# starkware-libs/stark-perpetual

Measured on AMD Instinct MI355X. Metric: pedersen_hashes_per_sec, higher is better.
Workload: dtype u32x9; 1 GPU; 2^16-leaf Pedersen Merkle rebuild per GPU (BASELINE.json configs[1]), 63 rebuilds in lockstep; tree_height=16, leaves_per_gpu=65536, calls_per_region=28, streams=2, window_bits=26, combine=none

## Files before the change

### stark-perpetual_amd/csrc/pedersen.hip

```cpp
#include <algorithm>
#include <cstdlib>
#include <cstring>
#include <map>
#include <vector>

#include "context.hpp"
#include "pedersen.hpp"
#include "quad.hpp"
#include "ragged_plan.hpp"

#ifndef SP_ACC_WAVES
#define SP_ACC_WAVES 1
#endif

namespace sp {

struct raw_aff {
  u256 x, y;
};
__device__ __forceinline__ raw_aff ld_raw(const aff_packed* e) {
  const uint4* q = reinterpret_cast<const uint4*>(e);
  const uint4 a = q[0], b = q[1], c = q[2], d = q[3];
  raw_aff r;
  r.x.w[0] = a.x; r.x.w[1] = a.y; r.x.w[2] = a.z; r.x.w[3] = a.w;
// ... 173 lines not shown
                      const int2* __restrict__ src, size_t plane) {
  bulk_accumulate(x, y, xstride, ystride, n, ped, w0, log2e, nwin, sX, sZZ, status, flag, src, plane,
                  (size_t)blockIdx.x * blockDim.x + threadIdx.x);
}

__device__ __forceinline__ fe shfl_xor_fe(const fe& v, int mask) {
  fe r;
#pragma unroll
  for (int i = 0; i < NL; ++i) r.l[i] = __shfl_xor(v.l[i], mask, 64);
  return r;
}
__device__ __forceinline__ uint32_t field_from_memory(const uint64_t* felt, int bit, int width) {
  const uint32_t* w = reinterpret_cast<const uint32_t*>(felt);
  const int wi = bit >> 5, sh = bit & 31;
  uint64_t two = (uint64_t)w[wi];
  if (wi + 1 < 8) two |= (uint64_t)w[wi + 1] << 32;
  return (uint32_t)(two >> sh) & ((1u << width) - 1u);
}
__device__ __forceinline__ uint32_t window_from_memory(const uint64_t* fx, const uint64_t* fy, int start,
                                                       int width) {
  if (start + width <= 252) return field_from_memory(fx, start, width);
  if (start >= 252) return field_from_memory(fy, start - 252, width);
  const int lo_n = 252 - start;
  return field_from_memory(fx, start, lo_n) | (field_from_memory(fy, 0, width - lo_n) << lo_n);
}

template <int LOG_L>
__device__ __forceinline__ xyzz split_accumulate(const uint64_t* fx, const uint64_t* fy, int sub,
                                                 const aff_packed* __restrict__ ped, int w0, int log2e,
                                                 int nwin) {
  constexpr int L = 1 << LOG_L;
  const int cnt_lo = nwin / L, extra = nwin % L;
  const int cnt = cnt_lo + (sub < extra ? 1 : 0);
  const int g0 = sub * cnt_lo + (sub < extra ? sub : extra);
  auto entry = [&](int g) {
    return window_entry(ped, g, window_from_memory(fx, fy, window_start(g, w0, log2e), window_width(g, w0, log2e)),
                        w0, log2e);
  };
  const window_ref r0 = entry(g0);
  const aff q0 = signed_aff(ld_raw(r0.entry), r0.negative);
  window_ref rn = entry(g0 + 1);
  raw_aff nxt = ld_raw(rn.entry);
  xyzz acc;
  {
    const aff q1 = signed_aff(nxt, rn.negative);
    if (cnt > 2) {
      rn = entry(g0 + 2);
      nxt = ld_raw(rn.entry);
    }
    acc = xyzz_mmadd<SP_SCAN_SPLIT>(q0, q1);
  }
  for (int j = 2; j < cnt; ++j) {
    const aff q = signed_aff(nxt, rn.negative);
    if (j + 1 < cnt) {
      rn = entry(g0 + j + 1);
      nxt = ld_raw(rn.entry);
    }
    acc = xyzz_madd<SP_SCAN_SPLIT>(acc, q);
  }
#pragma unroll 1
  for (int r = 0; r + 1 < LOG_L; ++r) {
    xyzz o;
    o.X = shfl_xor_fe(acc.X, 1 << r);
    o.Y = shfl_xor_fe(acc.Y, 1 << r);
    o.ZZ = shfl_xor_fe(acc.ZZ, 1 << r);
    o.ZZZ = shfl_xor_fe(acc.ZZZ, 1 << r);
    acc = xyzz_add<SP_SCAN_SPLIT>(acc, o);
  }
  if constexpr (LOG_L > 0) {
    constexpr int r = LOG_L - 1;
    xyzz o;
    o.X = shfl_xor_fe(acc.X, 1 << r);
    o.Y = shfl_xor_fe(acc.Y, 1 << r);
    o.ZZ = shfl_xor_fe(acc.ZZ, 1 << r);
    o.ZZZ = shfl_xor_fe(acc.ZZZ, 1 << r);
    fe X3, ZZ3;
    xyzz_add_x_only<SP_SCAN_SPLIT>(acc, o, X3, ZZ3);
    acc.X = X3;
    acc.ZZ = ZZ3;
  }
  return acc;
}

template <int LOG_L, bool FUSED>
__global__ void __launch_bounds__(256)
ped_accumulate_split_kernel(const uint64_t* __restrict__ x, const uint64_t* __restrict__ y, size_t xstride,
                            size_t ystride, size_t n, const aff_packed* __restrict__ ped, int w0, int log2e,
                            int nwin, int32_t* __restrict__ sX, int32_t* __restrict__ sZZ,
                            uint8_t* __restrict__ status, unsigned* __restrict__ flag,
                            const int2* __restrict__ src, uint64_t* __restrict__ out, size_t ostride,
                            size_t plane) {
  constexpr int L = 1 << LOG_L;
  const size_t gt = (size_t)blockIdx.x * blockDim.x + threadIdx.x;
  const size_t e_raw = gt >> LOG_L;
  const int sub = (int)(gt & (L - 1));
  const bool active = e_raw < n;
  const size_t e = active ? e_raw : n - 1;
  const uint64_t *fx, *fy;
  operand_pointers(x, y, xstride, ystride, src, e, fx, fy);
  const xyzz acc = split_accumulate<LOG_L>(fx, fy, sub, ped, w0, log2e, nwin);
  uint8_t st = SP_HASH_OK;
  u256 xa_plain;
  if (FUSED) {
    fe zz = acc.ZZ;
    if constexpr (LOG_L < 2) {
      if (fe_is_zero(zz)) {
        zz = FE_ONE_M;
        st = SP_HASH_UNHASHABLE;
      }
    }
    const fe zinv = fe_inv_shared_quad<(LOG_L >= 2 ? 0 : 2 - LOG_L), true>(zz, (int)(threadIdx.x & 3));
    if constexpr (LOG_L >= 2) {
      if (limbs_is_zero(zinv)) st = SP_HASH_UNHASHABLE;
    }
    xa_plain = fe_pack(fe_canon(fe_mul(acc.X, zinv)));
  }
  if (!active || sub != 0) return;
  if (!u256_lt(ld_u256(fx), U256_P) || !u256_lt(ld_u256(fy), U256_P)) st = SP_HASH_OUT_OF_RANGE;
  if (FUSED) {
    st_u256(out + 4 * e * ostride, xa_plain);
  } else {
    store_limbs(sX, plane, e, acc.X);
    store_limbs(sZZ, plane, e, acc.ZZ);
  }
  if (status) status[e] = st;
  if (st != SP_HASH_OK && flag) atomicOr(flag, (unsigned)st);
}

template <int LOG_L>
__global__ void __launch_bounds__(256, SP_ACC_WAVES)
ped_accumulate_mixed_kernel(const uint64_t* __restrict__ x, const uint64_t* __restrict__ y, size_t xstride,
                            size_t ystride, size_t n_bulk, size_t rem, unsigned bulk_blocks,
                            const aff_packed* __restrict__ ped, int w0, int log2e, int nwin,
                            int32_t* __restrict__ sX, int32_t* __restrict__ sZZ, uint8_t* __restrict__ status,
                            unsigned* __restrict__ flag, const int2* __restrict__ src, size_t plane) {
  if (blockIdx.x < bulk_blocks) {
    bulk_accumulate(x, y, xstride, ystride, n_bulk, ped, w0, log2e, nwin, sX, sZZ, status, flag, src, plane,
                    (size_t)blockIdx.x * blockDim.x + threadIdx.x);
    return;
  }
  constexpr int L = 1 << LOG_L;
  const size_t gt = (size_t)(blockIdx.x - bulk_blocks) * blockDim.x + threadIdx.x;
  const size_t e_raw = gt >> LOG_L;
  const int sub = (int)(gt & (L - 1));
  const bool active = e_raw < rem;
  const size_t e = n_bulk + (active ? e_raw : rem - 1);
  const uint64_t *fx, *fy;
  operand_pointers(x, y, xstride, ystride, src, e, fx, fy);
  const xyzz acc = split_accumulate<LOG_L>(fx, fy, sub, ped, w0, log2e, nwin);
  if (!active || sub != 0) return;
  uint8_t st = SP_HASH_OK;
  if (!u256_lt(ld_u256(fx), U256_P) || !u256_lt(ld_u256(fy), U256_P)) st = SP_HASH_OUT_OF_RANGE;
  store_limbs(sX, plane, e, acc.X);
  store_limbs(sZZ, plane, e, acc.ZZ);
  if (status) status[e] = st;
  if (st != SP_HASH_OK && flag) atomicOr(flag, (unsigned)st);
}

template <int LOG_Q, bool SPARSE>
__device__ __forceinline__ u256 quad_hash(const uint64_t* fx, const uint64_t* fy, int mode, const aff_packed* __restrict__ cpts,
                                          int cx, int cy, const aff_packed* __restrict__ ped, int w0, int log2e,
                                          int nwin_plan, int g, bool* unhashable) {
  constexpr int QUADS = 1 << LOG_Q;
  const int q = g >> 2, k = g & 3;
  int nwin = nwin_plan, first_real = 0;
  if constexpr (SPARSE) {
    nwin = mode == 0 ? nwin_plan : 1 + nwin_plan - (mode == 1 ? cx : cy);
    first_real = mode == 1 ? cx - 1 : (mode == 2 ? -1 : 0);
  }
  auto entry = [&](int v) {
    if constexpr (SPARSE) {
      if (mode != 0 && v == 0) return unpack_raw(ld_raw(cpts + (mode - 1)));
    }
    const int w = first_real + v;
    const window_ref r =
        window_entry(ped, w, window_from_memory(fx, fy, window_start(w, w0, log2e), window_width(w, w0, log2e)), w0, log2e);
    return signed_aff(ld_raw(r.entry), r.negative);
  };
  const int cnt = nwin / QUADS + (q < nwin % QUADS ? 1 : 0);
  int max_cnt = (nwin + QUADS - 1) / QUADS;
  if constexpr (SPARSE) {
    max_cnt = 0;
    if (__any(mode == 0)) max_cnt = (nwin_plan + QUADS - 1) / QUADS;
    if (__any(mode == 1)) max_cnt = max(max_cnt, (1 + nwin_plan - cx + QUADS - 1) / QUADS);
    if (__any(mode == 2)) max_cnt = max(max_cnt, (1 + nwin_plan - cy + QUADS - 1) / QUADS);
  }
  const bool upper = (k & 2) != 0;
  const bool odd = (k & 1) != 0;
  const int wa = (upper && cnt >= 3) ? q + 2 * QUADS : q;
  const int wb = (upper && cnt >= 4) ? q + 3 * QUADS : q + QUADS;
  const aff pa = entry(wa), pb = entry(wb);
  qpt p = qmmadd(pa.x, pa.y, pb.x, pb.y, k);
  if (upper && cnt == 3) {
    p.a = odd ? pa.y : pa.x;
    p.b = FE_ONE_M;
  }
  qpt s = qadd<false>(p, k);
  if (cnt == 2) {
    s.a = fe_dpp<quad_perm(0, 1, 0, 1)>(p.a);
// ... 194 lines not shown
    const u256 xa = quad_hash<LOG_Q, false>(fx, fy, 0, nullptr, 0, 0, ped, w0, log2e, nwin_plan, g, &unhashable);
    if (live && g == 0) {
      if (!u256_lt(ld_u256(w), U256_P) || (j == 0 && !u256_lt(ld_u256(h), U256_P))) st |= SP_HASH_OUT_OF_RANGE;
      else if (unhashable) st |= SP_HASH_UNHASHABLE;
    }
    __syncthreads();
    if (live && g == 0) {
      uint32_t* sl = reinterpret_cast<uint32_t*>(slot[grp]);
#pragma unroll
      for (int k = 0; k < 8; ++k) sl[k] = xa.w[k];
      if (j == steps - 1 && writer) {
        fold_result<SIDED>(e, xa, st, out, status, expect, estride, verdict);
        if (st != SP_HASH_OK && flag) atomicOr(flag, (unsigned)st);
      }
    }
    __syncthreads();
    h = slot[grp];
  }
}

__global__ void __launch_bounds__(256)
ped_fold_ragged_scatter_kernel(const uint64_t* __restrict__ work, const uint64_t* __restrict__ lone, bool sided,
                               const uint32_t* __restrict__ off, const uint32_t* __restrict__ perm,
                               const uint32_t* __restrict__ step_off, const uint8_t* __restrict__ step_status, size_t n,
                               unsigned* __restrict__ flag, uint8_t* __restrict__ status, uint64_t* __restrict__ out,
                               const uint64_t* __restrict__ expect, size_t estride, uint8_t* __restrict__ verdict) {
  const size_t k = (size_t)blockIdx.x * blockDim.x + threadIdx.x;
  if (k >= n) return;
  const uint32_t c = perm[k];
  const uint32_t o0 = off[c], steps = off[c + 1] - o0 - (sided ? 0 : 1);
  uint8_t st = SP_HASH_OK;
  u256 v;
  if (steps == 0) {
    v = ld_u256(lone + 4 * (size_t)(sided ? c : o0));
    if (!u256_lt(v, U256_P)) st = SP_HASH_OUT_OF_RANGE;
    if (st != SP_HASH_OK && flag) atomicOr(flag, (unsigned)st);
  } else {
    v = ld_u256(work + 4 * k);
    for (uint32_t s = 0; s < steps; ++s) st |= step_status[(size_t)step_off[s] + k];
  }
  fold_result<true>(c, v, st, out, status, expect, estride, verdict);
}

__global__ void __launch_bounds__(256)
ped_top_kernel(uint64_t* __restrict__ cur, size_t n_in, int n_levels, const aff_packed* __restrict__ ped, int w0, int log2e,
               int nwin_plan, unsigned* __restrict__ flag) {
  constexpr int LANES = 32, GROUPS = 256 / LANES;
  __shared__ uint64_t slot[2][GROUPS][4];
  const int g = (int)(threadIdx.x % LANES), grp = (int)(threadIdx.x / LANES);
  const size_t b = blockIdx.x;
  const int chunk = 1 << n_levels;
  uint64_t* out = cur + 4 * n_in;
  size_t n_out = n_in >> 1;
  int share = 4 - n_levels;
  for (int t = 0; t < n_levels; ++t, ++share) {
    const int cnt = chunk >> (t + 1);
    const int i = grp >> share;
    const bool writer = g == 0 && (grp & ((1 << share) - 1)) == 0;
    const uint64_t *fx, *fy;
    if (t == 0) {
      fx = cur + 4 * ((size_t)chunk * b + 2 * (size_t)i);
      fy = fx + 4;
    } else {
      fx = slot[(t - 1) & 1][2 * i];
      fy = slot[(t - 1) & 1][2 * i + 1];
    }
    bool unhashable;
    const u256 xa = quad_hash<3, false>(fx, fy, 0, nullptr, 0, 0, ped, w0, log2e, nwin_plan, g, &unhashable);
    uint8_t st = unhashable ? SP_HASH_UNHASHABLE : SP_HASH_OK;
    if (t == 0 && writer && (!u256_lt(ld_u256(fx), U256_P) || !u256_lt(ld_u256(fy), U256_P))) st = SP_HASH_OUT_OF_RANGE;
    if (writer) {
      uint32_t* sl = reinterpret_cast<uint32_t*>(slot[t & 1][i]);
#pragma unroll
      for (int w = 0; w < 8; ++w) sl[w] = xa.w[w];
      st_u256(out + 4 * ((size_t)cnt * b + (size_t)i), xa);
      if (st != SP_HASH_OK && flag) atomicOr(flag, (unsigned)st);
    }
    __syncthreads();
    out += 4 * n_out;
    n_out >>= 1;
  }
}

__global__ void __launch_bounds__(256)
ped_finish_kernel(const int32_t* __restrict__ sX, int32_t* __restrict__ sZZ, int32_t* __restrict__ sPre,
                  size_t n, size_t T, uint64_t* __restrict__ out, size_t ostride,
                  uint8_t* __restrict__ status, unsigned* __restrict__ flag) {
  const size_t t = (size_t)blockIdx.x * blockDim.x + threadIdx.x;
  if (t >= T) return;
  const size_t cnt = t < n ? (n - t + T - 1) / T : 0;
  fe run = FE_ONE_M;
  if (cnt > 0) {
    fe znext = load_limbs(sZZ, n, t);
#pragma unroll 1
    for (size_t j = 0; j < cnt; ++j) {
      const size_t e = t + j * T;
      const fe z = znext;
      if (j + 1 < cnt) znext = load_limbs(sZZ, n, e + T);
      store_limbs(sPre, n, e, run);
      run = fe_mul(run, z);
    }
  }
  if (fe_is_zero(run)) {
    run = FE_ONE_M;
#pragma unroll 1
    for (size_t e = t; e < n; e += T) {
      fe z = load_limbs(sZZ, n, e);
      if (fe_is_zero(z)) {
        z = FE_ONE_M;
        store_limbs(sZZ, n, e, z);
        if (status) status[e] = SP_HASH_UNHASHABLE;
        if (flag) atomicOr(flag, (unsigned)SP_HASH_UNHASHABLE);
      }
      store_limbs(sPre, n, e, run);
      run = fe_mul(run, z);
    }
  }
  size_t e = cnt > 0 ? t + (cnt - 1) * T : 0;
  fe zn = run, pn = run, xn = run;
  if (cnt > 0) {
    zn = load_limbs(sZZ, n, e);
    pn = load_limbs(sPre, n, e);
    xn = load_limbs(sX, n, e);
  }
  fe inv = fe_inv_shared_quad<2, true>(run, (int)(threadIdx.x & 3));
#pragma unroll 1
  for (size_t j = cnt; j-- > 0;) {
    const fe z = zn, pre = pn, xv = xn;
    const size_t cur = t + j * T;
    if (j > 0) {
      zn = load_limbs(sZZ, n, cur - T);
      pn = load_limbs(sPre, n, cur - T);
      xn = load_limbs(sX, n, cur - T);
    }
    const fe zinv = fe_mul(inv, pre);
    inv = fe_mul(inv, z);
    const fe xa = fe_mul(xv, zinv);
    st_u256(out + 4 * cur * ostride, fe_pack(fe_canon(xa)));
  }
}

template <bool Z_IN_LDS>
__global__ void __launch_bounds__(256)
ped_finish_lds_kernel(const int32_t* __restrict__ sX, int32_t* __restrict__ sZZ, size_t n, size_t T,
                      uint64_t* __restrict__ out, size_t ostride, uint8_t* __restrict__ status,
                      unsigned* __restrict__ flag, int kmax) {
  extern __shared__ int32_t fin_lds[];
  int32_t* lpre = fin_lds;
  int32_t* lz = fin_lds + (size_t)kmax * NL * 256;
  auto lds_put = [&](int32_t* base, size_t j, const fe& v) {
#pragma unroll
    for (int k = 0; k < NL; ++k) base[((j * NL + k) << 8) + threadIdx.x] = v.l[k];
  };
  auto lds_get = [&](const int32_t* base, size_t j) {
    fe v;
#pragma unroll
    for (int k = 0; k < NL; ++k) v.l[k] = base[((j * NL + k) << 8) + threadIdx.x];
    return v;
  };
  const size_t t = (size_t)blockIdx.x * blockDim.x + threadIdx.x;
  if (t >= T) return;
  const size_t cnt = t < n ? (n - t + T - 1) / T : 0;
  fe run = FE_ONE_M;
  if (cnt > 0) {
    fe znext = load_limbs(sZZ, n, t);
#pragma unroll 1
// ... 167 lines not shown
static int get_scratch_tail(size_t n, size_t tail_bytes, Scratch& s, char** tail, hipStream_t st) {
  DeviceBuffer& buf = g_stream_scratch[stream_key(st)];
  const size_t plane = ((9 * n * sizeof(int32_t)) + 255) & ~(size_t)255;
  SP_HIP(buf.reserve(3 * plane + 256 + tail_bytes));
  char* b = (char*)buf.ptr;
  s.X = (int32_t*)b;
  s.ZZ = (int32_t*)(b + plane);
  s.Pre = (int32_t*)(b + 2 * plane);
  s.flag = (unsigned*)(b + 3 * plane);
  if (tail) *tail = b + 3 * plane + 256;
  return SP_OK;
}
int get_scratch_public(size_t n, Scratch& s, hipStream_t st) { return get_scratch_tail(n, 0, s, nullptr, st); }

static size_t g_finish_lanes = getenv("STARKPERP_FINISH_LANES") ? (size_t)atoll(getenv("STARKPERP_FINISH_LANES")) : 65536;
static size_t parse_split_lanes() {
  const char* e = getenv("STARKPERP_SPLIT_LANES");
  long long v = e ? atoll(e) : 65536;
  if (v < 256) v = 256;
  if (v > (1ll << 24)) v = 1ll << 24;
  return ((size_t)v + 255) & ~(size_t)255;
}
static size_t g_split_lanes = parse_split_lanes();
static bool g_finish_lds = getenv("STARKPERP_NO_FINISH_LDS") == nullptr;
static int finish_lds_ready() {
  static std::map<int, int> done;
  int dev = -1;
  if (hipGetDevice(&dev) != hipSuccess) return SP_ERR_HIP;
  auto it = done.find(dev);
  if (it != done.end()) return it->second;
  const int want = 16 * NL * 256 * (int)sizeof(int32_t);
  hipError_t e = hipFuncSetAttribute(reinterpret_cast<const void*>(ped_finish_lds_kernel<true>),
                                     hipFuncAttributeMaxDynamicSharedMemorySize, want);
  if (e == hipSuccess)
    e = hipFuncSetAttribute(reinterpret_cast<const void*>(ped_finish_lds_kernel<false>),
                            hipFuncAttributeMaxDynamicSharedMemorySize, want);
  if (e != hipSuccess) (void)hipGetLastError();
  return done[dev] = (e == hipSuccess ? SP_OK : SP_ERR_HIP);
}
static size_t finish_threads(size_t n) {
  size_t K = (n + g_finish_lanes - 1) / g_finish_lanes;
  if (K < 1) K = 1;
  if (K > 32) K = 32;
  return ((n + K - 1) / K + 3) & ~(size_t)3;
}

void release_ragged_stage();
void release_pedersen_state() {
  for (auto& kv : g_stream_scratch) kv.second.release();
  g_stream_scratch.clear();
  release_ragged_stage();
  for (hipEvent_t e : g_prof.ev) (void)hipEventDestroy(e);
  g_prof.ev.clear();
  g_prof.units.clear();
  g_prof.used = 0;
  g_prof.enabled = false;
}

void constant_window_counts(const PedPlan& p, int& cx, int& cy) {
  cx = cy = 0;
  for (int g = 0; g < p.nwin; ++g) {
    if (p.start[g] + p.bits[g] <= 252) ++cx;
    if (p.start[g] >= 252) ++cy;
  }
}
static bool sparse_class(const PedPlan& plan, int log_q, int& cx, int& cy) {
  if (!g_sparse_enabled || (log_q != 1 && log_q != 2)) return false;
  constant_window_counts(plan, cx, cy);
  const int shortest = 1 + plan.nwin - (cx > cy ? cx : cy);
  return cx >= 1 && cy >= 1 && shortest >= (2 << log_q);
}
int enqueue_partial_points(const uint64_t* felts, int count, aff_packed* out, hipStream_t st, bool* usable) {
  Context& c = ctx();
  int cx, cy;
  constant_window_counts(c.plan, cx, cy);
  *usable = cx >= 1 && cy >= 1 && count > 0;
  if (!*usable) return SP_OK;
  hipLaunchKernelGGL(ped_partial_kernel, dim3((unsigned)((2 * count + 63) / 64)), dim3(64), 0, st, felts, count, c.ped,
                     (int)c.plan.bits[0], c.plan.log2e, c.plan.nwin, cx, cy, out);
  SP_HIP(hipGetLastError());
  return SP_OK;
}

static int enqueue_pedersen_impl(const uint64_t* x, size_t xs, const uint64_t* y, size_t ys, uint64_t* out,
                                 size_t os, uint8_t* status, unsigned* flag, size_t n, hipStream_t st,
                                 const Scratch& s, const int2* src, const aff_packed* cpts);
int enqueue_pedersen(const uint64_t* x, size_t xs, const uint64_t* y, size_t ys, uint64_t* out,
                     size_t os, uint8_t* status, unsigned* flag, size_t n, hipStream_t st,
                     const Scratch& s, const int2* src) {
  return enqueue_pedersen_impl(x, xs, y, ys, out, os, status, flag, n, st, s, src, nullptr);
}
int enqueue_pedersen_sparse(const uint64_t* x, const uint64_t* y, uint64_t* out, unsigned* flag, size_t n,
                            hipStream_t st, const Scratch& s, const int2* src, const aff_packed* cpts) {
  return enqueue_pedersen_impl(x, 1, y, 1, out, 1, nullptr, flag, n, st, s, src, cpts);
}
static bool g_path_fusion = getenv("STARKPERP_NO_PATH_FUSION") == nullptr;
static bool g_top_fusion = getenv("STARKPERP_NO_TOP_FUSION") == nullptr;
static bool g_chain_fusion = getenv("STARKPERP_NO_CHAIN_FUSION") == nullptr;
int enqueue_pedersen_chain(const uint64_t* first, const uint64_t* words, long long word_stride, size_t n, size_t steps,
                           bool h_right, uint64_t* out, unsigned* flag, hipStream_t st, bool* done) {
  *done = false;
  Context& c = ctx();
  const int w0 = c.plan.bits[0], log2e = c.plan.log2e, nwin = c.plan.nwin;
  if (!g_chain_fusion || n == 0 || steps < 2 || steps > 0x7fffffffull) return SP_OK;
  const QuadShape q = quad_shape(n, nwin);
  if (q.log_q == 0) return SP_OK;
  dispatch_quad(q.log_q, false, [&](auto Q, auto) {
    hipLaunchKernelGGL((ped_chain_kernel<decltype(Q)::value>), dim3(q.blocks), dim3(256), 0, st, first, words, word_stride,
                       n, (int)steps, h_right, c.ped, w0, log2e, nwin, flag, out, q.dup);
  });
  SP_HIP(hipGetLastError());
  *done = true;
  return SP_OK;
}
int enqueue_pedersen_top(uint64_t* cur, size_t n_in, unsigned remaining, unsigned* flag, hipStream_t st, int* levels_done) {
  *levels_done = 0;
  Context& c = ctx();
  const int nwin = c.plan.nwin;
  if (!g_top_fusion || !g_quad_enabled || nwin > 64 || nwin < 16 || remaining < 2 || n_in / 2 > g_quad_max || n_in < 4) return SP_OK;
  const int L = remaining < 4 ? (int)remaining : 4;
  const unsigned blocks = (unsigned)(n_in >> L);
  hipLaunchKernelGGL(ped_top_kernel, dim3(blocks), dim3(256), 0, st, cur, n_in, L, c.ped, (int)c.plan.bits[0], c.plan.log2e,
                     nwin, flag);
  SP_HIP(hipGetLastError());
  *levels_done = L;
  return SP_OK;
}
int enqueue_pedersen_path(uint64_t* felts, const uint64_t* emp, unsigned* flag, size_t n, hipStream_t st,
                          const int2* src_all, const PathLevels& pl, const aff_packed* cpts_tree, bool* done) {
  *done = false;
  Context& c = ctx();
  const int w0 = c.plan.bits[0], log2e = c.plan.log2e, nwin = c.plan.nwin;
  if (!g_path_fusion || n == 0 || pl.n_levels < 2) return SP_OK;
  const QuadShape q = quad_shape(n, nwin);
  if (q.log_q == 0) return SP_OK;
  int cx = 0, cy = 0;
  const bool sparse = cpts_tree != nullptr && sparse_class(c.plan, q.log_q, cx, cy);
  dispatch_quad(q.log_q, sparse, [&](auto Q, auto S) {
    hipLaunchKernelGGL((ped_path_kernel<decltype(Q)::value, decltype(S)::value>), dim3(q.blocks), dim3(256), 0, st, felts,
                       emp, n, c.ped, w0, log2e, nwin, flag, src_all, pl, q.dup, sparse ? cpts_tree : nullptr, cx, cy);
  });
  SP_HIP(hipGetLastError());
  *done = true;
  return SP_OK;
}

static int enqueue_pedersen_impl(const uint64_t* x, size_t xs, const uint64_t* y, size_t ys, uint64_t* out,
                                 size_t os, uint8_t* status, unsigned* flag, size_t n, hipStream_t st,
                                 const Scratch& s, const int2* src, const aff_packed* cpts) {
  if (n == 0) return SP_OK;
  Context& c = ctx();
  bool prof = false;
  const int w0 = c.plan.bits[0], log2e = c.plan.log2e, nwin = c.plan.nwin;
  int log_l = 0;
  bool fused = false;
  if (g_split_enabled) {
    if (n * 8 <= g_split_lanes) log_l = 3;
    else if (n * 4 <= g_split_lanes) log_l = 2;
    else if (n * 2 <= g_split_lanes) log_l = 1;
    while (log_l > 0 && nwin < (2 << log_l)) --log_l;
  }
  const QuadShape q = quad_shape(n, nwin);
  if (q.log_q != 0) {
    int cx = 0, cy = 0;
    const bool sparse = cpts != nullptr && src != nullptr && sparse_class(c.plan, q.log_q, cx, cy);
    dispatch_quad(q.log_q, sparse, [&](auto Q, auto S) {
      hipLaunchKernelGGL((ped_quad_kernel<decltype(Q)::value, decltype(S)::value>), dim3(q.blocks), dim3(256), 0, st, x, y,
                         xs, ys, n, c.ped, w0, log2e, nwin, status, flag, src, out, os, q.dup, cpts, cx, cy);
    });
    fused = true;
  } else if (log_l == 0 && !(g_split_enabled && g_fuse_enabled && n <= 65536)) {
    size_t n_bulk = n, rem = 0;
    int rem_l = 0;
    if (g_level_split && g_split_enabled && n > g_split_lanes && (n % g_split_lanes) != 0 &&
        (n % g_split_lanes) * 2 <= g_split_lanes) {
      rem = n % g_split_lanes;
      rem_l = rem * 8 <= g_split_lanes ? 3 : (rem * 4 <= g_split_lanes ? 2 : 1);
      while (rem_l > 0 && nwin < (2 << rem_l)) --rem_l;
      if (rem_l == 0) rem = 0;
      n_bulk = n - rem;
    }
    if (rem == 0) {
      prof = g_prof.enabled && g_prof.used + 2 <= g_prof.ev.size() && n > 65536;
      if (prof) (void)hipEventRecord(g_prof.ev[g_prof.used], st);
      hipLaunchKernelGGL(ped_accumulate_kernel, dim3((unsigned)((n_bulk + 255) / 256)), dim3(256), 0, st, x, y, xs, ys,
                         n_bulk, c.ped, w0, log2e, nwin, s.X, s.ZZ, status, flag, src, n);
    } else {
      const unsigned bulk_blocks = (unsigned)(n_bulk / 256);
      const unsigned rblocks = (unsigned)(((rem << rem_l) + 255) / 256);
#define SP_LAUNCH_MIXED(LOGL)                                                                                     \
  hipLaunchKernelGGL((ped_accumulate_mixed_kernel<LOGL>), dim3(bulk_blocks + rblocks), dim3(256), 0, st, x, y, xs, \
                     ys, n_bulk, rem, bulk_blocks, c.ped, w0, log2e, nwin, s.X, s.ZZ, status, flag, src, n)
      if (rem_l == 3) SP_LAUNCH_MIXED(3);
      else if (rem_l == 2) SP_LAUNCH_MIXED(2);
      else SP_LAUNCH_MIXED(1);
#undef SP_LAUNCH_MIXED
    }
    if (prof) {
      (void)hipEventRecord(g_prof.ev[g_prof.used + 1], st);
      g_prof.units.push_back(n);
      g_prof.used += 2;
    }
  } else {
    const unsigned blocks = (unsigned)(((n << log_l) + 255) / 256);
    fused = g_fuse_enabled && (n << log_l) <= 65536;
#define SP_LAUNCH_SPLIT(LOGL, FUSEDV)                                                                      \
  hipLaunchKernelGGL((ped_accumulate_split_kernel<LOGL, FUSEDV>), dim3(blocks), dim3(256), 0, st, x, y, xs, \
                     ys, n, c.ped, w0, log2e, nwin, s.X, s.ZZ, status, flag, src, out, os, n)
    if (log_l == 0) SP_LAUNCH_SPLIT(0, true);
    else if (log_l == 3) { if (fused) SP_LAUNCH_SPLIT(3, true); else SP_LAUNCH_SPLIT(3, false); }
    else if (log_l == 2) { if (fused) SP_LAUNCH_SPLIT(2, true); else SP_LAUNCH_SPLIT(2, false); }
    else { if (fused) SP_LAUNCH_SPLIT(1, true); else SP_LAUNCH_SPLIT(1, false); }
#undef SP_LAUNCH_SPLIT
  }
  if (!fused) {
    const size_t T = finish_threads(n);
    const unsigned tpb = T >= 256 ? 256 : 64;
    const unsigned blocksB = (unsigned)((T + tpb - 1) / tpb);
    const size_t kmax = (n + T - 1) / T;
    if (g_finish_lds && tpb == 256 && kmax >= 2 && kmax <= 16 && finish_lds_ready() == SP_OK) {
      const bool z_too = kmax <= 8;
      const size_t lds_bytes = kmax * NL * 256 * sizeof(int32_t) * (z_too ? 2 : 1);
      if (z_too) hipLaunchKernelGGL((ped_finish_lds_kernel<true>), dim3(blocksB), dim3(256), lds_bytes, st, s.X, s.ZZ, n, T,
                                    out, os, status, flag, (int)kmax);
      else hipLaunchKernelGGL((ped_finish_lds_kernel<false>), dim3(blocksB), dim3(256), lds_bytes, st, s.X, s.ZZ, n, T,
                              out, os, status, flag, (int)kmax);
    } else {
      hipLaunchKernelGGL(ped_finish_kernel, dim3(blocksB), dim3(tpb), 0, st, s.X, s.ZZ, s.Pre, n, T, out,
                         os, status, flag);
    }
  }
  SP_HIP(hipGetLastError());
  return SP_OK;
}

static bool g_chain_ragged = getenv("STARKPERP_NO_CHAIN_RAGGED") == nullptr;
static bool g_path_fold = getenv("STARKPERP_NO_PATH_FOLD") == nullptr;
struct RaggedStage {
  PinnedBuffer host;
  hipEvent_t copied = nullptr;
  bool pending = false;
};
static std::map<StreamKey, RaggedStage> g_ragged_stage;
void release_ragged_stage() {
// ... 383 lines not shown
  if (n != 0 && roots == nullptr) { set_error("merkle paths: roots must not be NULL"); return SP_ERR_BAD_ARGUMENT; }
  return merkle_paths_host(leaves, siblings, off, height, keys, n, nullptr, 0, roots, nullptr, status);
}
int sp_merkle_verify_paths(const uint64_t* leaves, const uint64_t* siblings, const uint32_t* off, unsigned height,
                           const uint64_t* keys, size_t n, const uint64_t* expected, size_t n_expected,
                           uint8_t* verdict, uint8_t* status) {
  if (n != 0 && (verdict == nullptr || expected == nullptr)) {
    set_error("merkle paths: expected and verdict must not be NULL");
    return SP_ERR_BAD_ARGUMENT;
  }
  if (n == 0 && verdict == nullptr) return SP_OK;
  return merkle_paths_host(leaves, siblings, off, height, keys, n, expected, n_expected, nullptr, verdict, status);
}

int sp_pedersen_chain(const uint64_t* elems, size_t n_elems, uint64_t* out, uint8_t* status) {
  SP_REQUIRE_READY();
  if (n_elems < 1) { set_error("chain needs at least one element"); return SP_ERR_BAD_ARGUMENT; }
  Context& c = ctx();
  ctx_lock lk(c.mu);
  SP_HIP(c.io.reserve(n_elems * 32 + 64));
  uint64_t* d_el = (uint64_t*)c.io.ptr;
  uint64_t* d_out = (uint64_t*)((char*)c.io.ptr + n_elems * 32);
  SP_HIP(hipMemcpy(d_el, elems, n_elems * 32, hipMemcpyHostToDevice));
  uint8_t st8 = 0;
  int rc = sp_pedersen_chains_dev(d_el, 1, n_elems, d_out, &st8, 0);
  if (rc != SP_OK) return rc;
  SP_HIP(hipDeviceSynchronize());
  SP_HIP(hipMemcpy(out, d_out, 32, hipMemcpyDeviceToHost));
  if (status) *status = st8;
  return SP_OK;
}

int sp_pedersen_chain_right(const uint64_t* elems, size_t n_elems, uint64_t* out, uint8_t* status) {
  SP_REQUIRE_READY();
  if (n_elems < 1) { set_error("chain needs at least one element"); return SP_ERR_BAD_ARGUMENT; }
  Context& c = ctx();
  ctx_lock lk(c.mu);
  SP_HIP(c.io.reserve((n_elems + 2) * 32 + 64));
  uint64_t* d_el = (uint64_t*)c.io.ptr;
  uint64_t* d_a = d_el + 4 * n_elems;
  uint64_t* d_b = d_a + 4;
  SP_HIP(hipMemcpy(d_el, elems, n_elems * 32, hipMemcpyHostToDevice));
  Scratch s;
  int rc = get_scratch(1, s, 0);
  if (rc != SP_OK) return rc;
  SP_HIP(hipMemsetAsync(s.flag, 0, sizeof(unsigned), 0));
  const uint64_t* h = d_el + 4 * (n_elems - 1);
  uint64_t* nxt = d_a;
  bool fused = false;
  if (n_elems >= 3) {
    rc = enqueue_pedersen_chain(h, d_el + 4 * (n_elems - 2), -1, 1, n_elems - 1, true, d_a, s.flag, 0, &fused);
    if (rc != SP_OK) return rc;
    if (fused) h = d_a;
  }
  for (size_t i = n_elems - 1; !fused && i-- > 0;) {
    rc = enqueue_pedersen(d_el + 4 * i, 1, h, 1, nxt, 1, nullptr, s.flag, 1, 0, s, nullptr);
    if (rc != SP_OK) return rc;
    h = nxt;
    nxt = (nxt == d_a) ? d_b : d_a;
  }
  SP_HIP(hipDeviceSynchronize());
  SP_HIP(hipMemcpy(out, h, 32, hipMemcpyDeviceToHost));
  if (status) {
    unsigned f = 0;
    SP_HIP(hipMemcpy(&f, s.flag, sizeof(unsigned), hipMemcpyDeviceToHost));
    *status = (uint8_t)f;
  }
  return SP_OK;
}

int sp_merkle_forest_dev(uint64_t* levels, size_t n_trees, unsigned height, uint8_t* status,
                         void* stream) {
  CtxByPointer sp_ctx_sel__(levels);
  SP_REQUIRE_READY();
  if (n_trees == 0) return SP_OK;
  if (height > 40 || (n_trees >> (40 - height)) != 0) { set_error("forest too large"); return SP_ERR_BAD_ARGUMENT; }
  Context& c = ctx();
  ctx_lock lk(c.mu);
  hipStream_t st = (hipStream_t)stream;
  const size_t n0 = n_trees << height;
  Scratch s;
  int rc = get_scratch(n0 / 2 + 1, s, st);
  if (rc != SP_OK) return rc;
  SP_HIP(hipMemsetAsync(s.flag, 0, sizeof(unsigned), st));
  uint64_t* cur = levels;
  size_t n = n0;
  for (unsigned k = 0; k < height;) {
    int fused = 0;
    rc = enqueue_pedersen_top(cur, n, height - k, s.flag, st, &fused);
    if (rc != SP_OK) return rc;
    if (fused > 0) {
      for (int j = 0; j < fused; ++j, n >>= 1) cur += 4 * n;
      k += (unsigned)fused;
      continue;
    }
    uint64_t* nxt = cur + 4 * n;
    rc = enqueue_pedersen(cur, 2, cur + 4, 2, nxt, 1, nullptr, s.flag, n / 2, st, s, nullptr);
    if (rc != SP_OK) return rc;
    cur = nxt;
    ++k;
    n >>= 1;
  }
  if (status) SP_HIP(hipMemcpyAsync(status, s.flag, 1, hipMemcpyDeviceToHost, st));
  return SP_OK;
}

int sp_merkle_build_dev(uint64_t* levels, unsigned height, uint8_t* status, void* stream) {
  return sp_merkle_forest_dev(levels, 1, height, status, stream);
}

int sp_commit_rows_dev(const uint64_t* cols, size_t n_rows, size_t n_cols, uint64_t* levels, uint8_t* status,
                       void* stream) {
  CtxByPointer sp_ctx_sel__(cols);
  SP_REQUIRE_READY();
  if (n_rows == 0 || (n_rows & (n_rows - 1)) != 0 || n_cols == 0) {
    set_error("rows must be a power of two, columns at least one");
    return SP_ERR_BAD_ARGUMENT;
  }
  ctx_lock lk(ctx().mu);
  unsigned height = 0;
  while (((size_t)1 << height) < n_rows) ++height;
  uint8_t st_chain = 0, st_tree = 0;
  int rc = sp_pedersen_chains_dev(cols, n_rows, n_cols, levels, status ? &st_chain : nullptr, stream);
  if (rc != SP_OK) return rc;
  rc = sp_merkle_build_dev(levels, height, status ? &st_tree : nullptr, stream);
  if (rc != SP_OK) return rc;
  if (status) {
    SP_HIP(hipStreamSynchronize((hipStream_t)stream));
    *status = st_chain | st_tree;
  }
  return SP_OK;
}

int sp_merkle_root(const uint64_t* leaves, unsigned height, uint64_t* root, uint64_t* levels_out,
                   uint8_t* status) {
  SP_REQUIRE_READY();
  if (height > 30) { set_error("height too large"); return SP_ERR_BAD_ARGUMENT; }
  Context& c = ctx();
  const size_t n0 = (size_t)1 << height;
  const size_t total = 2 * n0 - 1;
  ctx_lock lk(c.mu);
  SP_HIP(c.io.reserve(total * 32));
  uint64_t* d = (uint64_t*)c.io.ptr;
  SP_HIP(hipMemcpy(d, leaves, n0 * 32, hipMemcpyHostToDevice));
  uint8_t st8 = 0;
  int rc = sp_merkle_build_dev(d, height, &st8, 0);
  if (rc != SP_OK) return rc;
  SP_HIP(hipDeviceSynchronize());
  SP_HIP(hipMemcpy(root, d + 4 * (total - 1), 32, hipMemcpyDeviceToHost));
  if (levels_out) SP_HIP(hipMemcpy(levels_out, d, total * 32, hipMemcpyDeviceToHost));
  if (status) *status = st8;
  return SP_OK;
}

}
```

Baseline: 1.032 billion hashes/s.

## Fuse the lower Merkle levels into one tail kernel with per-level lane classes

Adds ped_tail_kernel. It computes several consecutive Merkle levels in one launch, passes intermediate hashes through double-buffered shared memory, and picks split-accumulate or quad-hash lane widths per level as the tree narrows. The goal is to cut per-level kernel launches and global round trips in the small-n part of each rebuild. It also skips the flag memset and the error atomics when no status is requested. In exchange, lane utilisation per level is fixed by block shape, and the take-condition depends on lane-class heuristics matching at every level.

```diff
diff --git a/stark-perpetual_amd/csrc/pedersen.hip b/stark-perpetual_amd/csrc/pedersen.hip
--- a/stark-perpetual_amd/csrc/pedersen.hip
+++ b/stark-perpetual_amd/csrc/pedersen.hip
@@ -279,6 +279,22 @@
   return acc;
 }
 
+template <int LOG_L>
+__device__ __forceinline__ u256 split_fused_x(const xyzz& acc, uint8_t* st) {
+  fe zz = acc.ZZ;
+  if constexpr (LOG_L < 2) {
+    if (fe_is_zero(zz)) {
+      zz = FE_ONE_M;
+      *st = SP_HASH_UNHASHABLE;
+    }
+  }
+  const fe zinv = fe_inv_shared_quad<(LOG_L >= 2 ? 0 : 2 - LOG_L), true>(zz, (int)(threadIdx.x & 3));
+  if constexpr (LOG_L >= 2) {
+    if (limbs_is_zero(zinv)) *st = SP_HASH_UNHASHABLE;
+  }
+  return fe_pack(fe_canon(fe_mul(acc.X, zinv)));
+}
+
 template <int LOG_L, bool FUSED>
 __global__ void __launch_bounds__(256)
 ped_accumulate_split_kernel(const uint64_t* __restrict__ x, const uint64_t* __restrict__ y, size_t xstride,
@@ -298,20 +314,7 @@
   const xyzz acc = split_accumulate<LOG_L>(fx, fy, sub, ped, w0, log2e, nwin);
   uint8_t st = SP_HASH_OK;
   u256 xa_plain;
-  if (FUSED) {
-    fe zz = acc.ZZ;
-    if constexpr (LOG_L < 2) {
-      if (fe_is_zero(zz)) {
-        zz = FE_ONE_M;
-        st = SP_HASH_UNHASHABLE;
-      }
-    }
-    const fe zinv = fe_inv_shared_quad<(LOG_L >= 2 ? 0 : 2 - LOG_L), true>(zz, (int)(threadIdx.x & 3));
-    if constexpr (LOG_L >= 2) {
-      if (limbs_is_zero(zinv)) st = SP_HASH_UNHASHABLE;
-    }
-    xa_plain = fe_pack(fe_canon(fe_mul(acc.X, zinv)));
-  }
+  if (FUSED) xa_plain = split_fused_x<LOG_L>(acc, &st);
   if (!active || sub != 0) return;
   if (!u256_lt(ld_u256(fx), U256_P) || !u256_lt(ld_u256(fy), U256_P)) st = SP_HASH_OUT_OF_RANGE;
   if (FUSED) {
@@ -672,6 +675,66 @@
   }
 }
 
+template <int S>
+__device__ __forceinline__ u256 tail_hash(const uint64_t* fx, const uint64_t* fy, int lane, const aff_packed* __restrict__ ped,
+                                          int w0, int log2e, int nwin, uint8_t* st) {
+  if constexpr (S < 3) {
+    return split_fused_x<S>(split_accumulate<S>(fx, fy, lane, ped, w0, log2e, nwin), st);
+  } else {
+    bool unhashable;
+    const u256 xa = quad_hash<S - 2, false>(fx, fy, 0, nullptr, 0, 0, ped, w0, log2e, nwin, lane, &unhashable);
+    if (unhashable) *st = SP_HASH_UNHASHABLE;
+    return xa;
+  }
+}
+
+__global__ void __launch_bounds__(256)
+ped_tail_kernel(uint64_t* __restrict__ cur, size_t n_in, int s0, int n_levels, const aff_packed* __restrict__ ped, int w0,
+                int log2e, int nwin_plan, unsigned* __restrict__ flag) {
+  __shared__ uint64_t slot[2][256][4];
+  const size_t b = blockIdx.x;
+  const int tid = (int)threadIdx.x;
+  uint64_t* out = cur + 4 * n_in;
+  size_t n_out = n_in >> 1;
+#pragma unroll 1
+  for (int t = 0; t < n_levels; ++t) {
+    const int s = s0 + t;
+    const int cls = s < 5 ? s : 5;
+    const int cnt = 256 >> s;
+    const int i = tid >> s, lane = tid & ((1 << cls) - 1);
+    const bool writer = (tid & ((1 << s) - 1)) == 0;
+    const uint64_t *fx, *fy;
+    if (t == 0) {
+      fx = cur + 4 * (2 * (size_t)cnt * b + 2 * (size_t)i);
+      fy = fx + 4;
+    } else {
+      fx = slot[(t - 1) & 1][2 * i];
+      fy = slot[(t - 1) & 1][2 * i + 1];
+    }
+    uint8_t st = SP_HASH_OK;
+    u256 xa;
+    switch (cls) {
+      case 0: xa = tail_hash<0>(fx, fy, lane, ped, w0, log2e, nwin_plan, &st); break;
+      case 1: xa = tail_hash<1>(fx, fy, lane, ped, w0, log2e, nwin_plan, &st); break;
+      case 2: xa = tail_hash<2>(fx, fy, lane, ped, w0, log2e, nwin_plan, &st); break;
+      case 3: xa = tail_hash<3>(fx, fy, lane, ped, w0, log2e, nwin_plan, &st); break;
+      case 4: xa = tail_hash<4>(fx, fy, lane, ped, w0, log2e, nwin_plan, &st); break;
+      default: xa = tail_hash<5>(fx, fy, lane, ped, w0, log2e, nwin_plan, &st); break;
+    }
+    if (t == 0 && writer && (!u256_lt(ld_u256(fx), U256_P) || !u256_lt(ld_u256(fy), U256_P))) st = SP_HASH_OUT_OF_RANGE;
+    if (writer) {
+      uint32_t* sl = reinterpret_cast<uint32_t*>(slot[t & 1][i]);
+#pragma unroll
+      for (int w = 0; w < 8; ++w) sl[w] = xa.w[w];
+      st_u256(out + 4 * ((size_t)cnt * b + (size_t)i), xa);
+      if (st != SP_HASH_OK && flag) atomicOr(flag, (unsigned)st);
+    }
+    __syncthreads();
+    out += 4 * n_out;
+    n_out >>= 1;
+  }
+}
+
 __global__ void __launch_bounds__(256)
 ped_finish_kernel(const int32_t* __restrict__ sX, int32_t* __restrict__ sZZ, int32_t* __restrict__ sPre,
                   size_t n, size_t T, uint64_t* __restrict__ out, size_t ostride,
@@ -1005,6 +1068,24 @@
   return SP_OK;
 }
 
+static int split_log_l(size_t n, int nwin) {
+  int log_l = 0;
+  if (g_split_enabled) {
+    if (n * 8 <= g_split_lanes) log_l = 3;
+    else if (n * 4 <= g_split_lanes) log_l = 2;
+    else if (n * 2 <= g_split_lanes) log_l = 1;
+    while (log_l > 0 && nwin < (2 << log_l)) --log_l;
+  }
+  return log_l;
+}
+static int tail_lane_class(size_t n, int nwin) {
+  const QuadShape q = quad_shape(n, nwin);
+  if (q.log_q != 0) return 2 + q.log_q;
+  const int log_l = split_log_l(n, nwin);
+  const bool one_launch = g_split_enabled && g_fuse_enabled && log_l <= 2 && (n << log_l) <= 65536;
+  return one_launch ? log_l : -1;
+}
+
 static int enqueue_pedersen_impl(const uint64_t* x, size_t xs, const uint64_t* y, size_t ys, uint64_t* out,
                                  size_t os, uint8_t* status, unsigned* flag, size_t n, hipStream_t st,
                                  const Scratch& s, const int2* src, const aff_packed* cpts);
@@ -1019,6 +1100,7 @@
 }
 static bool g_path_fusion = getenv("STARKPERP_NO_PATH_FUSION") == nullptr;
 static bool g_top_fusion = getenv("STARKPERP_NO_TOP_FUSION") == nullptr;
+static bool g_tail_fusion = getenv("STARKPERP_NO_TAIL_FUSION") == nullptr;
 static bool g_chain_fusion = getenv("STARKPERP_NO_CHAIN_FUSION") == nullptr;
 int enqueue_pedersen_chain(const uint64_t* first, const uint64_t* words, long long word_stride, size_t n, size_t steps,
                            bool h_right, uint64_t* out, unsigned* flag, hipStream_t st, bool* done) {
@@ -1040,6 +1122,19 @@
   *levels_done = 0;
   Context& c = ctx();
   const int nwin = c.plan.nwin;
+  if (g_tail_fusion && nwin >= 16 && nwin <= 64 && n_in >= 2) {
+    const int s0 = tail_lane_class(n_in / 2, nwin);
+    const int L = 9 - s0;
+    bool take = s0 >= 0 && s0 <= 4 && remaining >= (unsigned)L;
+    for (int t = 1; take && t < L; ++t) take = tail_lane_class(n_in >> (t + 1), nwin) == (s0 + t < 5 ? s0 + t : 5);
+    if (take) {
+      hipLaunchKernelGGL(ped_tail_kernel, dim3((unsigned)(n_in >> L)), dim3(256), 0, st, cur, n_in, s0, L, c.ped,
+                         (int)c.plan.bits[0], c.plan.log2e, nwin, flag);
+      SP_HIP(hipGetLastError());
+      *levels_done = L;
+      return SP_OK;
+    }
+  }
   if (!g_top_fusion || !g_quad_enabled || nwin > 64 || nwin < 16 || remaining < 2 || n_in / 2 > g_quad_max || n_in < 4) return SP_OK;
   const int L = remaining < 4 ? (int)remaining : 4;
   const unsigned blocks = (unsigned)(n_in >> L);
@@ -1075,14 +1170,8 @@
   Context& c = ctx();
   bool prof = false;
   const int w0 = c.plan.bits[0], log2e = c.plan.log2e, nwin = c.plan.nwin;
-  int log_l = 0;
+  const int log_l = split_log_l(n, nwin);
   bool fused = false;
-  if (g_split_enabled) {
-    if (n * 8 <= g_split_lanes) log_l = 3;
-    else if (n * 4 <= g_split_lanes) log_l = 2;
-    else if (n * 2 <= g_split_lanes) log_l = 1;
-    while (log_l > 0 && nwin < (2 << log_l)) --log_l;
-  }
   const QuadShape q = quad_shape(n, nwin);
   if (q.log_q != 0) {
     int cx = 0, cy = 0;
@@ -1632,12 +1721,13 @@
   Scratch s;
   int rc = get_scratch(n0 / 2 + 1, s, st);
   if (rc != SP_OK) return rc;
-  SP_HIP(hipMemsetAsync(s.flag, 0, sizeof(unsigned), st));
+  unsigned* flag = status ? s.flag : nullptr;
+  if (flag) SP_HIP(hipMemsetAsync(flag, 0, sizeof(unsigned), st));
   uint64_t* cur = levels;
   size_t n = n0;
   for (unsigned k = 0; k < height;) {
     int fused = 0;
-    rc = enqueue_pedersen_top(cur, n, height - k, s.flag, st, &fused);
+    rc = enqueue_pedersen_top(cur, n, height - k, flag, st, &fused);
     if (rc != SP_OK) return rc;
     if (fused > 0) {
       for (int j = 0; j < fused; ++j, n >>= 1) cur += 4 * n;
@@ -1645,13 +1735,13 @@
       continue;
     }
     uint64_t* nxt = cur + 4 * n;
-    rc = enqueue_pedersen(cur, 2, cur + 4, 2, nxt, 1, nullptr, s.flag, n / 2, st, s, nullptr);
+    rc = enqueue_pedersen(cur, 2, cur + 4, 2, nxt, 1, nullptr, flag, n / 2, st, s, nullptr);
     if (rc != SP_OK) return rc;
     cur = nxt;
     ++k;
     n >>= 1;
   }
-  if (status) SP_HIP(hipMemcpyAsync(status, s.flag, 1, hipMemcpyDeviceToHost, st));
+  if (status) SP_HIP(hipMemcpyAsync(status, flag, 1, hipMemcpyDeviceToHost, st));
   return SP_OK;
 }
 
```

After: 1.048 billion hashes/s (median of 6 runs). 1.02x the previous value.
